# clayne/CPU-Raytracer

Measured on AMD Instinct MI355X. Metric: Mrays/s (primary+shadow+reflection+refraction), higher is better.
Workload: dtype f32

## Files before the change

cpu-raytracer_amd/csrc/rtx_api.hip:

```cpp
#include <hip/hip_runtime.h>
#include <stdio.h>
#include <stdlib.h>
#include <string.h>
#include <math.h>
#include <string>
#include <vector>
#include <algorithm>
#include <type_traits>

#include "../../include/rtx.h"
#include "rtx_device.h"
#include "rtx_math.h"
#include "rtx_libm.h"
#include "rtx_texture.h"
#include "rtx_trace.h"
#include "rtx_shade.h"
#include "rtx_packet.h"
#include "rtx_present.h"
#include "rtx_update.h"
#include "rtx_refit.h"
#include "rtx_build.h"
#include "rtx_normals.h"
#include "rtx_query.h"
#include "rtx_nearest.h"
// ... 31 lines not shown
    hipStream_t stream = nullptr;
    hipStream_t own_stream = nullptr;
    hipStream_t any_stream = nullptr;
    hipEvent_t ev_shade0 = nullptr, ev_shade_last = nullptr, ev_any_done = nullptr;
    void * ext_rgb = nullptr, * ext_packed = nullptr;
    std::string err;
    int n_cu = 0;

    struct BlasRefit { std::vector<int32_t> map4, map4c; bool bound = false; int32_t vertex_count = 0; DevBuf block; DevRefit dev; float * planes[3] = { nullptr, nullptr, nullptr }; void * sort_tmp = nullptr; size_t sort_bytes = 0; };
    struct BlasBuild { bool allocated = false; DevBuf block; DevBuild dev; void * sort_tmp = nullptr; size_t sort_bytes = 0; int levels = 0; };
    struct BlasNormals { bool allocated = false, set = false; DevBuf block; DevNormals dev; void * sort_tmp = nullptr; size_t sort_bytes = 0; unsigned int key_bits = 0; };
    struct BlasSide { bool allocated = false; DevBuf block; DevSide dev; };
    struct BlasHost { std::vector<DevBuf> arrays; int max_local_material = -1, inner_depth = -1; bool packet_ok = true; BlasRefit refit; BlasBuild build; BlasNormals normals; BlasSide side; };
    std::vector<DevBlas> h_blas;
    std::vector<BlasHost> blas;
    DevBuf d_blas, d_materials, d_textures, d_sky, d_ewa;
    std::vector<DevTexture> h_tex;
    std::vector<DevBuf> tex_texels;
    struct TexUpdate { bool allocated = false; rtxt::Plan plan; };
    std::vector<TexUpdate> tex_update;
    DevBuf d_srgb_lut;
    bool sky_uploaded = false;
    int material_count = 0, sky_size = 0;
    std::vector<rtx_material> h_materials; int tlas_inner_depth = -1; std::vector<int> frame_primitive_materials; bool refs_dirty = true; Knobs knobs; int item_blocks = 0, item_cap_alloc = 0; DevBuf d_pk_items, d_pk_item_count;

    DevBuf d_frame;
    StageRing frame_ring;
    DevScene scene;
    bool frame_set = false;
    bool frame_rigid = true;
    LoneFacts frame_lone = { false, false };
    DevBuf d_upd, d_upd_sort; int upd_cap = 0;
    DevBuf d_views, d_vfb_rgb, d_vfb_packed;
    StageRing view_ring;
    int32_t view_count = 0, vfb_cap = 0, ext_vcap = 0;
    void * ext_vrgb = nullptr, * ext_vpacked = nullptr;
    DevBuf d_rays;
    StageRing ray_ring;
    int32_t ray_count = 0, ext_ray_count = 0;
    const void * ext_rays = nullptr;
    uint32_t aov_channels = 0; bool aov_ext = false; int64_t aov_ext_cap = 0; DevAov aov_ext_ptrs = {};
    DevBuf d_aov[8]; int64_t aov_own_cap[8] = {};

    DevQueues q;
    DevBuf qb[20];
    DevBuf d_query[4], d_query_counters, d_query_heads; int32_t query_cap = 0;
    DevBuf d_query_sort; int32_t query_sort_cap = 0; size_t query_sort_tmp = 0;
// ... 119 lines not shown
        if (fc > 0.0) c->pk_blocks_closest = ((int)(c->n_cu * fc) + 1) & ~1;
    }
    {
        const int g = RTX_PK_CLASSES * RTX_WAVE / RTX_PK_BLOCK > 1 ? RTX_PK_CLASSES * RTX_WAVE / RTX_PK_BLOCK : 1;
        c->pk_blocks_any = (c->pk_blocks_any + g - 1) / g * g; c->pk_blocks_closest = (c->pk_blocks_closest + g - 1) / g * g;
        if (c->pk_blocks_any < g) c->pk_blocks_any = g;
        if (c->pk_blocks_closest < g) c->pk_blocks_closest = g;
    }
    long long max_threads = (long long)(c->trace_blocks_closest > c->trace_blocks_any ? c->trace_blocks_closest : c->trace_blocks_any) * RTX_TRACE_BLOCK;
    if ((long long)c->trace_blocks_count * RTX_TRACE_BLOCK > max_threads) max_threads = (long long)c->trace_blocks_count * RTX_TRACE_BLOCK;
    if ((long long)c->pk_blocks_any * RTX_PK_BLOCK > max_threads) max_threads = (long long)c->pk_blocks_any * RTX_PK_BLOCK;
    if ((long long)c->pk_blocks_closest * RTX_PK_BLOCK > max_threads) max_threads = (long long)c->pk_blocks_closest * RTX_PK_BLOCK;
    c->q.pk_defer_t0 = (int)knob_int("RTX_PK_DEFER", 8, 0, 64);
    c->q.pk_defer_leaf = (int)knob_int("RTX_PK_DEFER_LEAF", c->q.pk_defer_t0 / 2, 0, 64);
    c->q.pk_defer_t0_closest = (int)knob_int("RTX_PK_DEFER_CLOSEST", 64, 0, 64);
    c->q.pk_closest_asm = (int)knob_int("RTX_PK_CLOSEST_ASM", 1, 0, 1);
    c->q.pk_defer_t0_primary = (int)knob_int("RTX_PK_DEFER_PRIMARY", c->q.pk_closest_asm ? 4 : 64, 0, 64);
    c->q.pk_order = (int)knob_int("RTX_PK_ORDER", 1, 0, 1);
    c->q.prof_level = (int)knob_int("RTX_LANE_PROF_LEVEL", 2, 0, 100 + RTX_MAX_LEVELS);
    c->q.pk_defer_grow = (int)knob_int("RTX_PK_GROW", 3, 0, 31);
    c->q.spill_threads = (int)max_threads;
    rc = ensure(c, c->d_spill, (size_t)c->q.spill_threads * (RTX_MAX_STACK - RTX_LDS_STACK) * 4 * 3);
    if (!rc) rc = ensure(c, c->d_pk_fifo, (size_t)c->q.spill_threads * RTX_PK_FIFO * 8);
    { int ib = 0; hipOccupancyMaxActiveBlocksPerMultiprocessor(&ib, k_items, RTX_ITEM_BLOCK, 0); c->item_blocks = c->n_cu * (ib > 0 ? ib : 4);
      const double f = knob_real("RTX_ITEM_GRID", 0.0, 0.05, 64.0); if (f > 0.0) c->item_blocks = (int)(c->n_cu * f) > 0 ? (int)(c->n_cu * f) : 1; }
    c->q.pk_items = nullptr; c->q.pk_item_count = nullptr; c->q.pk_item_cap = 0;
    if (rc) { rtx_destroy(c); return rc; }
    bind_tables(c);
    *out_ctx = c;
    return RTX_OK;
}

extern "C" int rtx_destroy(rtx_ctx * c) {
    if (!c) return RTX_ERR_INVALID_ARG;
    hipSetDevice(c->cfg.device);
    if (c->stream) hipStreamSynchronize(c->stream);
    for (hipEvent_t e : c->event_pool) hipEventDestroy(e);
    if (c->graph_exec) { hipGraphExecDestroy(c->graph_exec); c->graph_exec = nullptr; }
    if (c->order_stream) { hipStreamSynchronize(c->order_stream); hipStreamDestroy(c->order_stream); hipEventDestroy(c->ev_cost); hipEventDestroy(c->ev_order); }
    if (c->any_stream) { hipStreamSynchronize(c->any_stream); hipStreamDestroy(c->any_stream); }
    if (c->ev_shade0) hipEventDestroy(c->ev_shade0);
    if (c->ev_shade_last) hipEventDestroy(c->ev_shade_last);
    if (c->ev_any_done) hipEventDestroy(c->ev_any_done);
    if (c->own_stream) hipStreamDestroy(c->own_stream);
    delete c;
    return RTX_OK;
}
// ... 976 lines not shown
        case SHADE_AOV_COUNT: hipLaunchKernelGGL((k_shade<true, false, VW, true, DevAov>),  g, b, 0, c->stream, sc, q, level, aov_t); break;
        case SHADE_AOV_CULL:  hipLaunchKernelGGL((k_shade<false, true, VW, true, DevAov>),  g, b, 0, c->stream, sc, q, level, aov_t); break;
        case SHADE_AOV:       hipLaunchKernelGGL((k_shade<false, false, VW, true, DevAov>), g, b, 0, c->stream, sc, q, level, aov_t); break;
        case SHADE_COUNT:     hipLaunchKernelGGL((k_shade<true, false, VW>),  g, b, 0, c->stream, sc, q, level); break;
        case SHADE_CULL:      hipLaunchKernelGGL((k_shade<false, true, VW>),  g, b, 0, c->stream, sc, q, level); break;
        default:              hipLaunchKernelGGL((k_shade<false, false, VW>), g, b, 0, c->stream, sc, q, level); break;
        }
    }); });
}

static void launch_any(rtx_ctx * c, const AnyLaunch & a, const DevScene & sc, const DevQueues & q) {
    const hipStream_t st = a.stream ? c->any_stream : c->stream;
    const dim3 plain(c->trace_blocks_count), lane(c->trace_blocks_any), tb(RTX_TRACE_BLOCK), pk(c->pk_blocks_any), pb(RTX_PK_BLOCK);
    launch_timed(c, "k_trace_any", st, [&] {
        switch (a.kernel) {
        case ANY_PLAIN_COUNT:   hipLaunchKernelGGL((k_trace<true, true>),   plain, tb, 0, st, sc, q, a.lo); break;
        case ANY_PLAIN:         hipLaunchKernelGGL((k_trace<true, false>),  plain, tb, 0, st, sc, q, a.lo); break;
        case ANY_LANE:          hipLaunchKernelGGL((k_trace_fast<true>),    lane, tb, 0, st, sc, q, a.lo, a.hi); break;
        case ANY_PACKET_STATS:  hipLaunchKernelGGL((k_packet<true, true>),  pk, pb, 0, st, sc, q, a.lo, a.hi); break;
        case ANY_PACKET_SPLIT:  hipLaunchKernelGGL((k_packet<true, false, true>), pk, pb, 0, st, sc, q, a.lo, a.hi); break;
        default:                hipLaunchKernelGGL((k_packet<true, false>), pk, pb, 0, st, sc, q, a.lo, a.hi); break;
        }
    });
    if (a.items) launch_timed(c, "k_trace_items", st, [&] { hipLaunchKernelGGL(k_items, dim3(c->item_blocks), dim3(RTX_ITEM_BLOCK), 0, st, sc, q, c->pk_blocks_any * (RTX_PK_BLOCK / RTX_WAVE), a.lo); });
}

static int run_batch(rtx_ctx * c, const RenderPlan & plan, const DevScene & sc, const DevQueues & q, const DevAov & aov_t, bool first_batch) {
    begin_batch(c, q.counters, q.pk_heads, (uint32_t)q.primary_slots, plan.plain != 0, first_batch);
    if (plan.heatmap) {
        launch_closest(c, plan, sc, q, 0);
        launch_timed(c, "k_heatmap", c->stream, [&] { with_views(plan.views, [&](auto V) { if constexpr (decltype(V)::value != RTX_CAM_RAYS) hipLaunchKernelGGL((k_heatmap<decltype(V)::value>), dim3(plan.stream_blocks), dim3(256), 0, c->stream, sc, q); }); });
        return RTX_OK;
    }
    int next_any = 0;
    for (int level = 0; level < plan.levels; level++) {
        launch_closest(c, plan, sc, q, level);
        if (plan.lpt && level == 0) {
            HIP_OK(c, hipEventRecord(c->ev_cost, c->stream)); HIP_OK(c, hipStreamWaitEvent(c->order_stream, c->ev_cost, 0));
            hipLaunchKernelGGL(k_packet_order, dim3(1), dim3(1024), 0, c->order_stream, (const uint32_t *)c->d_pk_cost.p, (uint32_t *)c->d_pk_order.p, plan.lpt_n);
            HIP_OK(c, hipEventRecord(c->ev_order, c->order_stream));
            c->lpt_valid = true;
        }
        launch_shade(c, plan, sc, q, aov_t, level);
        bool joined = false;
        for (; next_any < plan.n_any && plan.any[next_any].after_level == level; next_any++) {
            if (plan.any[next_any].stream && !joined) {
                const hipEvent_t ev = level == 0 ? c->ev_shade0 : c->ev_shade_last;
// ... 421 lines not shown
    if (rc) return rc;
    hipLaunchKernelGGL(k_debug_texture, dim3((n + 255) / 256), dim3(256), 0, c->stream, sc, texture_id, (const float *)din.p, (float *)dout.p, n);
    HIP_OK(c, hipStreamSynchronize(c->stream));
    HIP_OK(c, hipMemcpy(out3, dout.p, (size_t)n * 12, hipMemcpyDeviceToHost));
    return RTX_OK;
}

__global__ void k_debug_sky(const float * sky, int size, const float * dirs, float * out3, int n) {
    const int i = blockIdx.x * blockDim.x + threadIdx.x;
    if (i >= n) return;
    const v3 r = sky_sample(sky, size, V3(dirs[3 * i], dirs[3 * i + 1], dirs[3 * i + 2]));
    out3[3 * i] = r.x; out3[3 * i + 1] = r.y; out3[3 * i + 2] = r.z;
}

extern "C" int rtx_debug_blas_wide(rtx_ctx * c, int32_t blas_id, int32_t * stack_need) {
    if (!c || !stack_need || blas_id < 0 || (size_t)blas_id >= c->h_blas.size() || !c->h_blas[blas_id].nodes) return RTX_ERR_INVALID_ARG;
    *stack_need = c->h_blas[blas_id].pk4_nodes ? c->h_blas[blas_id].pk4_need : -1;
    return RTX_OK;
}

extern "C" int rtx_debug_blas_wide_closest(rtx_ctx * c, int32_t blas_id, int32_t * stack_need) {
    if (!c || !stack_need || blas_id < 0 || (size_t)blas_id >= c->h_blas.size() || !c->h_blas[blas_id].nodes) return RTX_ERR_INVALID_ARG;
    *stack_need = c->h_blas[blas_id].pk4c_nodes ? c->h_blas[blas_id].pk4c_need : -1;
    return RTX_OK;
}

extern "C" int rtx_debug_grids(rtx_ctx * c, int32_t out[8]) {
    if (!c || !out) return RTX_ERR_INVALID_ARG;
    out[0] = c->n_cu; out[1] = c->trace_blocks_closest; out[2] = c->trace_blocks_any; out[3] = c->trace_blocks_count;
    out[4] = c->pk_blocks_closest; out[5] = c->pk_blocks_any; out[6] = c->item_blocks; out[7] = c->q.spill_threads;
    return RTX_OK;
}

extern "C" int rtx_debug_sky_sample(rtx_ctx * c, const float * dirs3, float * out3, int32_t n) {
    if (!c || !dirs3 || !out3 || n <= 0) return RTX_ERR_INVALID_ARG;
    hipSetDevice(c->cfg.device);
    DevBuf din, dout;
    int rc = upload(c, din, dirs3, (size_t)n * 12);
    if (!rc) rc = ensure(c, dout, (size_t)n * 12);
    if (rc) return rc;
    hipLaunchKernelGGL(k_debug_sky, dim3((n + 255) / 256), dim3(256), 0, c->stream, (const float *)c->d_sky.p, c->sky_size, (const float *)din.p, (float *)dout.p, n);
    HIP_OK(c, hipStreamSynchronize(c->stream));
    HIP_OK(c, hipMemcpy(out3, dout.p, (size_t)n * 12, hipMemcpyDeviceToHost));
    return RTX_OK;
}

// ... 841 lines not shown
```

cpu-raytracer_amd/csrc/rtx_device.h:

```cpp
#pragma once
#include <hip/hip_runtime.h>
#include <stdint.h>
#include "../../include/rtx.h"
#include "rtx_limits.h"

typedef float rtx_f4v __attribute__((ext_vector_type(4)));
typedef const __attribute__((address_space(1))) rtx_f4v * rtx_gptr;
#define RTX_GPTR(p) ((rtx_gptr)(const void *)(p))
static __device__ __forceinline__ float4 gld(rtx_gptr p, int i) { const rtx_f4v v = p[i]; return make_float4(v.x, v.y, v.z, v.w); }
typedef float rtx_f3v __attribute__((ext_vector_type(3)));
static __device__ __forceinline__ float3 gld3(rtx_gptr p, int i) {
    const rtx_f3v v = *(const __attribute__((address_space(1))) rtx_f3v *)(p + i);
    return make_float3(v.x, v.y, v.z);
}

#define RTX_TRI_STRIDE  4
#ifndef RTX_LDS_STACK
#define RTX_LDS_STACK    16
#endif
#define RTX_TRACE_BLOCK  256

#define PRIM_NONE     0
#define PRIM_TRI      (1 << 28)
#define PRIM_SPHERE   (2 << 28)
// ... 103 lines not shown
    int32_t *     pk_fifo;
    int32_t       prof_level;
    int32_t       pk_order;
    int32_t       pk_defer_grow;
    int32_t       pk_closest_asm;
    int32_t       pk_defer_t0_primary;
    int32_t       pk_defer_t0_closest;
    int32_t       pk_defer_t0;
    int32_t       pk_defer_leaf;
    int32_t       pk_item_cap;
    uint4 *       pk_items;
    uint32_t *    pk_item_count;
    DevCounters * counters;
    uint32_t *    stats_partial;
    int32_t       stats_stride;
    int32_t       stats_n[RTX_MAX_LEVELS + 1];
    uint32_t *       pk_cost;
    const uint32_t * pk_lpt_order;
    uint32_t *    pk_heads;
    uint32_t *    tm_packed;
    int32_t       tm_base;
    float *       fb_rgb;
    uint32_t *    fb_packed;
};
```

cpu-raytracer_amd/csrc/rtx_packet.h:

```cpp
#pragma once
#include "rtx_math.h"
#include "rtx_device.h"
#include "rtx_trace.h"
#include "rtx_shade.h"

#define RTX_PK_CLASSES  8
#ifndef RTX_PK_WAVES_ANY
#define RTX_PK_WAVES_ANY 5
#endif
#ifndef RTX_PK_WAVES_SPLIT
#define RTX_PK_WAVES_SPLIT 5
#endif
#ifndef RTX_PK_WAVES_CLOSEST
#define RTX_PK_WAVES_CLOSEST 4
#endif
#ifndef RTX_PK_CHUNK
#define RTX_PK_CHUNK 64u
#endif
#ifndef RTX_PK_WAVES_FUSED
#define RTX_PK_WAVES_FUSED 3
#endif

typedef const __attribute__((address_space(4))) rtx_f4v * rtx_cptr;
typedef float rtx_f2v __attribute__((ext_vector_type(2)));
// ... 1752 lines not shown
    if (lane == 0) for (int i = 0; i < 10; i++) { if (i == 4 || i == 5 || i == 7 || i == 8 || i == 9) atomicMax(&ctr->work[(ANY ? 0 : 10) + i], W.prof[i]); else atomicAdd(&ctr->work[(ANY ? 0 : 10) + i], W.prof[i]); }
#endif
#ifdef RTX_LANE_PROF
    if (!ANY && level == q.prof_level % 100 && lane == 0 && (W.lp[12] > 0u || (q.prof_level >= 100 && lp_had_packet))) {
        for (int i = 0; i < 10; i++) atomicAdd(&ctr->work[i], (unsigned long long)W.lp[i]);
        atomicMax(&ctr->work[10], (unsigned long long)W.lp[10]); atomicMax(&ctr->work[11], (unsigned long long)W.lp[11]); atomicAdd(&ctr->work[12], (unsigned long long)W.lp[12]);
        atomicMax(&ctr->work[13], __builtin_amdgcn_s_memtime() - lp_k0);
        atomicAdd(&ctr->work[14], __builtin_amdgcn_s_memtime() - lp_k0);
        atomicAdd(&ctr->work[15], 1ull);
        atomicAdd(&ctr->work[16], __builtin_amdgcn_s_memrealtime() - lp_r0);
        atomicAdd(&ctr->work[17], (unsigned long long)W.lp[13]); atomicAdd(&ctr->work[18], (unsigned long long)W.lp[14]);
        atomicAdd(&ctr->work[19], (unsigned long long)W.lp[15]);
    }
#endif
    if (ANY && SPLIT && q.pk_items && lane == 0) { q.pk_item_count[gwave] = (uint32_t)W.item_n; if ((uint32_t)W.item_n > __hip_atomic_load(&ctr->item_max[level], __ATOMIC_RELAXED, __HIP_MEMORY_SCOPE_AGENT)) atomicMax(&ctr->item_max[level], (uint32_t)W.item_n); }
    if (W.err) { if (lane == 0) atomicOr(&ctr->error_flags, ERR_STACK_OVERFLOW); }
    if (PSTAT && lane == 0) {
        atomicAdd(&ctr->work[15 + PKS_PACKETS], st_packets); atomicAdd(&ctr->work[15 + PKS_PAIR_STEPS], W.st_pairs);
        atomicAdd(&ctr->work[15 + PKS_TRI_STEPS], W.st_tris); atomicAdd(&ctr->work[15 + PKS_PAIR_LANES], W.st_pair_lanes);
        atomicAdd(&ctr->work[15 + PKS_TRI_LANES], W.st_tri_lanes);
    }
}

#define RTX_ITEM_LDS 8
#ifndef RTX_ITEM_BLOCK
#define RTX_ITEM_BLOCK 64
#endif
#define RTX_ITEM_MESHES 32
#ifndef RTX_ITEM_WAVES
#define RTX_ITEM_WAVES 6
#endif
__global__ __launch_bounds__(RTX_ITEM_BLOCK, RTX_ITEM_WAVES)
void k_items(const DevScene sc, const DevQueues q, const int n_chunks, const int level) {
    __shared__ int s_stk[RTX_ITEM_LDS][RTX_ITEM_BLOCK];
    __shared__ unsigned long long s_mesh[RTX_ITEM_MESHES][2];
    for (int b = threadIdx.x; b < RTX_ITEM_MESHES && b < sc.blas_count; b += blockDim.x) { s_mesh[b][0] = (unsigned long long)sc.blas[b].pk4_nodes; s_mesh[b][1] = (unsigned long long)sc.blas[b].tri_hot; }
    __syncthreads();
    const uint32_t gwave = (uint32_t)rfl((int)(blockIdx.x * (RTX_ITEM_BLOCK / RTX_WAVE) + (threadIdx.x >> 6)));
    const uint32_t n_batches = ((uint32_t)rfl((int)q.counters->item_max[level]) + 63u) >> 6;
    const uint32_t nwaves = gridDim.x * (RTX_ITEM_BLOCK / RTX_WAVE), units = (uint32_t)n_chunks * n_batches;
    int ovf[RTX_PK4_MAX_NEED + 4];
#ifdef RTX_ITEM_STATS
    unsigned long long st_iters = 0, st_busy = 0, st_batches = 0, st_items = 0;
#endif
    uint32_t u = gwave, pos = 0, lim = 0; const uint4 * items = q.pk_items;
    auto next_unit = [&]() {
        for (; u < units; u += nwaves) {
            const uint32_t chunk = u % (uint32_t)n_chunks, first = (u / (uint32_t)n_chunks) * 64u;
            const uint32_t n = (uint32_t)rfl((int)q.pk_item_count[chunk]);
            if (first < n) { pos = first; lim = first + 64u < n ? first + 64u : n; items = q.pk_items + 3 * (size_t)chunk * (size_t)q.pk_item_cap; u += nwaves; return true; }
        }
        return false;
    };
    bool have_unit = next_unit();
    bool busy = false, have_cur = false; uint32_t slot = 0; int psp = 0, cur_first = 0, cur_cnt = 0;
    v3 co = V3(0.0f, 0.0f, 0.0f), cd = V3(1.0f, 1.0f, 1.0f);
    PkRay ray; pk_set_ray(ray, co, cd, cd); ray.tcur = 0.0f;
    rtx_gptr nodes4 = nullptr, tris = nullptr;
    auto push = [&](int e) { if (psp < RTX_ITEM_LDS) s_stk[psp][threadIdx.x] = e; else if (psp < RTX_ITEM_LDS + RTX_PK4_MAX_NEED + 4) ovf[psp - RTX_ITEM_LDS] = e; psp++; };
    for (;;) {
        const unsigned long long idle = __ballot(!busy);
        if (idle != 0ull && have_unit) {
            const uint32_t rank = (uint32_t)__builtin_amdgcn_mbcnt_hi((uint32_t)(idle >> 32), __builtin_amdgcn_mbcnt_lo((uint32_t)idle, 0u));
            const uint32_t take = (uint32_t)__popcll(idle), avail = lim - pos;
            if (!busy && rank < avail) {
                const uint4 * const it = items + 3 * (size_t)(pos + rank);
                const uint4 q0 = it[0], q1 = it[1]; const uint2 q2 = *(const uint2 *)(it + 2);
                slot = q1.w;
                if (q2.y < RTX_ITEM_MESHES) { nodes4 = (rtx_gptr)s_mesh[q2.y][0]; tris = (rtx_gptr)s_mesh[q2.y][1]; }
                else { const DevBlas & B = sc.blas[q2.y]; nodes4 = RTX_GPTR(B.pk4_nodes); tris = RTX_GPTR(B.tri_hot); }
                co = V3(as_f((int)q0.x), as_f((int)q0.y), as_f((int)q0.z)); cd = V3(as_f((int)q1.x), as_f((int)q1.y), as_f((int)q1.z));
                pk_set_ray(ray, co, cd, vrcp(cd)); ray.tcur = as_f((int)q0.w);
                cur_first = rtxl::wide_first((int)q2.x); cur_cnt = rtxl::wide_count((int)q2.x); have_cur = true; psp = 0;
                busy = q.socc[slot] == 0u;
#ifdef RTX_ITEM_STATS
                st_items++;
#endif
            }
            pos += take < avail ? take : avail;
            if (pos >= lim) have_unit = next_unit();
        }
        if (__ballot(busy) == 0ull) { if (!have_unit) break; else continue; }
#ifdef RTX_ITEM_STATS
        st_iters++; st_busy += (unsigned long long)__popcll(__ballot(busy));
#endif
        if (busy && have_cur && cur_cnt == 0) {
            const Pk4Step s = pk4_step(nodes4, cur_first, ray);
            if (s.q3) push(s.e3);
            if (s.q2) push(s.e2);
            if (s.q1) push(s.e1);
            have_cur = s.have_cur; cur_first = s.cur_first; cur_cnt = s.cur_cnt;
        }
        if (busy && have_cur && cur_cnt > 0) {
            have_cur = false;
            for (int t = cur_first; t < cur_first + cur_cnt; t++) {
                const float4 p0 = gld(tris, RTX_TRI_STRIDE * t), e1 = gld(tris, RTX_TRI_STRIDE * t + 1), e2 = gld(tris, RTX_TRI_STRIDE * t + 2);
                float tt, uu, vv;
                if (tri_test(v3q(p0), v3q(e1), v3q(e2), co, cd, ray.tcur, tt, uu, vv)) { q.socc[slot] = 1u; busy = false; break; }
            }
        }
        if (busy && !have_cur) {
            if (psp == 0) busy = false;
            else {
                psp--;
                const int e = psp < RTX_ITEM_LDS ? s_stk[psp][threadIdx.x] : ovf[psp - RTX_ITEM_LDS];
                cur_first = rtxl::wide_first(e); cur_cnt = rtxl::wide_count(e); have_cur = true;
            }
        }
    }
#ifdef RTX_ITEM_STATS
    if ((threadIdx.x & 63) == 0) { atomicAdd(&q.counters->work[16], st_iters); atomicAdd(&q.counters->work[17], st_busy); atomicMax(&q.counters->work[19], st_iters); }
    atomicAdd(&q.counters->work[15], st_items);
#endif
}
```

cpu-raytracer_amd/csrc/rtx_plan.h:

```cpp
#pragma once
#include <stdint.h>
#include <string.h>
#include "../../include/rtx.h"
#include "rtx_limits.h"

struct Knobs {
    long long slot_budget;
    long long item_bytes_max;
    int shade_grid;
    int lane_from_level;
    int lane_from_level_any;
    int split_items;
    int resolve_block;
    int pk4_order;
    bool merge_any, no_wide, no_wide_closest, fail_item_alloc, graph; int lpt;
    bool fuse_shade;
    int update_small_max;
    int tex_pass_levels;
    bool lone_entry;
};

struct LoneFacts { bool lone, copy_class; };
static inline LoneFacts plan_lone_facts(int instance_count, const rtx_bvh_node * tlas_nodes, int tlas_node_count, const int32_t * tlas_indices, int tlas_index_count,
                                        const rtx_instance * instances) {
    LoneFacts f = { false, false };
    if (instance_count != 1 || tlas_node_count < 1 || tlas_index_count < 1 || !tlas_nodes || !tlas_indices || !instances) return f;
    if (tlas_nodes[0].count != 1 || tlas_nodes[0].left_or_first != 0 || tlas_indices[0] != 0) return f;
    f.lone = true;
    uint32_t bits[12]; memcpy(bits, instances[0].world_inv, sizeof(bits));
    f.copy_class = true;
    for (int k = 0; k < 12; k++) {
        const bool diagonal = k == 0 || k == 5 || k == 10;
        if (diagonal ? bits[k] != 0x3f800000u : (bits[k] & 0x7fffffffu) != 0u) f.copy_class = false;
    }
    return f;
}

struct StackFigures { bool unfit_mesh; int dt, blas_any, blas_shared; };

static inline bool plan_can_spawn(const rtx_material * materials, size_t count) {
    for (size_t i = 0; i < count; i++)
        for (int a = 0; a < 3; a++) if (materials[i].reflection[a] != 0.0f || materials[i].transmittance[a] != 0.0f) return true;
// ... 143 lines not shown
```

cpu-raytracer_amd/pyrtx/api.py:

```python
from __future__ import annotations

import ctypes as C
import os
from typing import Dict, List, Optional

import numpy as np

from . import scene_io as sio
from .ctypes_structs import RtxConfig, RtxFrame, RtxStats, RtxWork, RtxTextureDesc, RtxAovBuffers, RtxRay, RtxQueryFilter, AOV_CHANNELS, RTX_AOV_ALL, fill_frame

_HERE = os.path.dirname(os.path.abspath(__file__))
LIB_PATH = os.path.join(_HERE, "..", "csrc", "librtx_hip.so")

EXPORTS = ["rtx_abi_version", "rtx_create", "rtx_destroy", "rtx_last_error", "rtx_upload_blas", "rtx_upload_materials",
           "rtx_upload_texture", "rtx_upload_sky", "rtx_set_frame", "rtx_render_tiles", "rtx_synchronize", "rtx_get_stats",
           "rtx_read_framebuffer", "rtx_framebuffer_device_ptrs", "rtx_last_kernel_times", "rtx_enable_kernel_timing",
           "rtx_bind_framebuffer", "rtx_set_stream", "rtx_present", "rtx_debug_libm", "rtx_debug_texture_sample", "rtx_debug_sky_sample", "rtx_debug_blas_wide", "rtx_debug_blas_wide_closest",
           "rtx_group_unique_id", "rtx_group_create", "rtx_group_render", "rtx_group_destroy", "rtx_group_attach", "rtx_group_create_local", "rtx_group_render_local",
           "rtx_group_layout", "rtx_group_slot_pixels", "rtx_debug_group_loopback", "rtx_debug_trace_rays", "rtx_debug_occluded", "rtx_debug_light_plot",
           "rtx_set_views", "rtx_render_views", "rtx_read_views", "rtx_bind_view_framebuffer", "rtx_bind_aovs", "rtx_read_aovs",
           "rtx_set_rays", "rtx_bind_rays", "rtx_render_rays", "rtx_update_instances", "rtx_read_frame_state",
           "rtx_bind_blas_vertices", "rtx_refit_blas", "rtx_read_blas", "rtx_alloc_blas", "rtx_build_blas",
           "rtx_query_closest", "rtx_query_occluded", "rtx_debug_query_order", "rtx_debug_read_layouts",
           "rtx_alloc_texture", "rtx_update_texture", "rtx_read_texture", "rtx_update_sky",
           "rtx_alloc_blas_topology", "rtx_set_blas_topology", "rtx_blas_vertex_normals", "rtx_query_nearest", "rtx_query_hits", "rtx_query_sweep",
           "rtx_debug_grids", "rtx_set_object_masks", "rtx_update_object_masks", "rtx_read_object_masks",
           "rtx_query_nearest_filtered", "rtx_query_hits_filtered", "rtx_query_sweep_filtered",
           "rtx_blas_pseudonormals", "rtx_read_blas_pseudonormals", "rtx_query_signed_distance",
           "rtx_query_overlap", "rtx_query_overlap_filtered", "rtx_query_sweep_box", "rtx_query_sweep_box_filtered",
           "rtx_query_overlap_capsule", "rtx_query_overlap_capsule_filtered"]
VIEW_EXPORTS = ("rtx_set_views", "rtx_render_views", "rtx_read_views", "rtx_bind_view_framebuffer")
AOV_EXPORTS = ("rtx_bind_aovs", "rtx_read_aovs")
RAY_EXPORTS = ("rtx_set_rays", "rtx_bind_rays", "rtx_render_rays")
UPDATE_EXPORTS = ("rtx_update_instances", "rtx_read_frame_state")
REFIT_EXPORTS = ("rtx_bind_blas_vertices", "rtx_refit_blas", "rtx_read_blas")
BUILD_EXPORTS = ("rtx_alloc_blas", "rtx_build_blas")
QUERY_EXPORTS = ("rtx_query_closest", "rtx_query_occluded")
QUERY_SORT_EXPORTS = ("rtx_debug_query_order",)
LAYOUT_EXPORTS = ("rtx_debug_read_layouts",)
TEXTURE_EXPORTS = ("rtx_alloc_texture", "rtx_update_texture", "rtx_read_texture", "rtx_update_sky")
NORMALS_EXPORTS = ("rtx_alloc_blas_topology", "rtx_set_blas_topology", "rtx_blas_vertex_normals")
NEAREST_EXPORTS = ("rtx_query_nearest",)
SIGNED_EXPORTS = ("rtx_blas_pseudonormals", "rtx_read_blas_pseudonormals", "rtx_query_signed_distance")
HITS_EXPORTS = ("rtx_query_hits",)
SWEEP_EXPORTS = ("rtx_query_sweep",)
GRID_EXPORTS = ("rtx_debug_grids",)
MASK_EXPORTS = ("rtx_set_object_masks", "rtx_update_object_masks", "rtx_read_object_masks",
                "rtx_query_nearest_filtered", "rtx_query_hits_filtered", "rtx_query_sweep_filtered")
OVERLAP_EXPORTS = ("rtx_query_overlap", "rtx_query_overlap_filtered")
SWEEP_BOX_EXPORTS = ("rtx_query_sweep_box", "rtx_query_sweep_box_filtered")
OVERLAP_CAPSULE_EXPORTS = ("rtx_query_overlap_capsule", "rtx_query_overlap_capsule_filtered")
OPTIONAL_EXPORTS = (OVERLAP_CAPSULE_EXPORTS + SWEEP_BOX_EXPORTS + OVERLAP_EXPORTS + VIEW_EXPORTS + AOV_EXPORTS + RAY_EXPORTS + UPDATE_EXPORTS + REFIT_EXPORTS + QUERY_EXPORTS + QUERY_SORT_EXPORTS + LAYOUT_EXPORTS
                    + TEXTURE_EXPORTS + NORMALS_EXPORTS + NEAREST_EXPORTS + HITS_EXPORTS + SWEEP_EXPORTS + GRID_EXPORTS + MASK_EXPORTS + SIGNED_EXPORTS)
RTX_QUERY_MAX_HITS = 8
RTX_TEXELS_RGB_F32 = 0
RTX_TEXELS_RGBA8_SRGB = 1
RTX_UPDATE_MAX_INSTANCES = 65536
RTX_ERR_STATE = 5

RTX_RENDER_COUNT_WORK = 1
RTX_RENDER_SIMPLE_TRACE = 2
RTX_RENDER_CULL_DEAD_SHADOW_RAYS = 4
RTX_RENDER_SERIAL = 8
RTX_RENDER_LANE_TRACE = 16
RTX_RENDER_PACKET_STATS = 32
RTX_RENDER_PACKET_CLOSEST = 64
RTX_RENDER_AOV = 128
RTX_MAX_VIEWS = 4096
RTX_QUERY_DISTANCE = 1
RTX_QUERY_POSITION = 2
RTX_QUERY_NORMAL = 4
RTX_QUERY_UV = 16
RTX_QUERY_MATERIAL_ID = 32
RTX_QUERY_OBJECT_ID = 64
RTX_QUERY_TRIANGLE_ID = 128
# ... 93 lines not shown
        lib.rtx_build_blas.argtypes = [vp, i32, vp, vp, vp, vp, vp]
    if hasattr(lib, "rtx_query_closest"):
        lib.rtx_query_closest.argtypes = [vp, vp, C.c_int64, u32, C.POINTER(RtxQueryBuffers), u32]
        lib.rtx_query_occluded.argtypes = [vp, vp, C.c_int64, vp, u32]
    if hasattr(lib, "rtx_query_nearest"):
        lib.rtx_query_nearest.argtypes = [vp, vp, C.c_int64, u32, C.POINTER(RtxQueryBuffers), u32]
    if hasattr(lib, "rtx_query_sweep"):
        lib.rtx_query_sweep.argtypes = [vp, vp, C.c_int64, u32, C.POINTER(RtxQueryBuffers), u32]
    if hasattr(lib, "rtx_query_hits"):
        lib.rtx_query_hits.argtypes = [vp, vp, C.c_int64, i32, u32, C.POINTER(RtxQueryBuffers), vp, u32]
    if hasattr(lib, "rtx_set_object_masks"):
        lib.rtx_set_object_masks.argtypes = [vp, vp, i32]
        lib.rtx_update_object_masks.argtypes = [vp, vp, i32]
        lib.rtx_read_object_masks.argtypes = [vp, vp, i32, C.POINTER(i32)]
        lib.rtx_query_nearest_filtered.argtypes = [vp, vp, C.c_int64, u32, C.POINTER(RtxQueryBuffers), u32, C.POINTER(RtxQueryFilter)]
        lib.rtx_query_sweep_filtered.argtypes = [vp, vp, C.c_int64, u32, C.POINTER(RtxQueryBuffers), u32, C.POINTER(RtxQueryFilter)]
        lib.rtx_query_hits_filtered.argtypes = [vp, vp, C.c_int64, i32, u32, C.POINTER(RtxQueryBuffers), vp, u32, C.POINTER(RtxQueryFilter)]
    if hasattr(lib, "rtx_debug_query_order"):
        lib.rtx_debug_query_order.argtypes = [vp, vp, i32, C.c_int64, vp]
    if hasattr(lib, "rtx_debug_read_layouts"):
        lib.rtx_debug_read_layouts.argtypes = [vp, i32, vp, vp, vp, vp, vp, vp, vp]
    if hasattr(lib, "rtx_debug_grids"):
        lib.rtx_debug_grids.argtypes = [vp, vp]
    if hasattr(lib, "rtx_update_texture"):
        lib.rtx_alloc_texture.argtypes = [vp, i32, i32, i32, i32]
        lib.rtx_update_texture.argtypes = [vp, i32, vp, i32]
        lib.rtx_read_texture.argtypes = [vp, i32, C.POINTER(RtxTextureDesc), vp, C.c_int64]
        lib.rtx_update_sky.argtypes = [vp, vp, i32]
    if hasattr(lib, "rtx_blas_vertex_normals"):
        lib.rtx_alloc_blas_topology.argtypes = [vp, i32, i32, i32]
        lib.rtx_set_blas_topology.argtypes = [vp, i32, vp]
        lib.rtx_blas_vertex_normals.argtypes = [vp, i32, vp, vp]
    if hasattr(lib, "rtx_query_signed_distance"):
        lib.rtx_blas_pseudonormals.argtypes = [vp, i32, vp]
        lib.rtx_read_blas_pseudonormals.argtypes = [vp, i32, vp, vp]
        lib.rtx_query_signed_distance.argtypes = [vp, vp, C.c_int64, u32, C.POINTER(RtxQueryBuffers), vp, vp, u32, C.POINTER(RtxQueryFilter)]
    if hasattr(lib, "rtx_query_overlap"):
        lib.rtx_query_overlap.argtypes = [vp, vp, C.c_int64, i32, vp, vp, vp, u32]
        lib.rtx_query_overlap_filtered.argtypes = [vp, vp, C.c_int64, i32, vp, vp, vp, u32, C.POINTER(RtxQueryFilter)]
    if hasattr(lib, "rtx_query_overlap_capsule"):
        lib.rtx_query_overlap_capsule.argtypes = [vp, vp, C.c_int64, i32, vp, vp, vp, u32]
        lib.rtx_query_overlap_capsule_filtered.argtypes = [vp, vp, C.c_int64, i32, vp, vp, vp, u32, C.POINTER(RtxQueryFilter)]
    if hasattr(lib, "rtx_query_sweep_box"):
        lib.rtx_query_sweep_box.argtypes = [vp, vp, C.c_int64, vp, vp, vp, vp, vp, u32]
        lib.rtx_query_sweep_box_filtered.argtypes = [vp, vp, C.c_int64, vp, vp, vp, vp, vp, u32, C.POINTER(RtxQueryFilter)]
    for name in EXPORTS:
# ... 761 lines not shown
    def debug_read_layouts(self, blas_id: int = -1) -> Dict:
        info = np.zeros(8, np.int32)
        self._chk(self.lib.rtx_debug_read_layouts(self.ctx, int(blas_id), info.ctypes.data, None, None, None, None, None, None), "rtx_debug_read_layouts")
        n = int(info[0])
        pk = np.zeros((n, 8), np.uint32)
        if blas_id < 0:
            self._chk(self.lib.rtx_debug_read_layouts(self.ctx, int(blas_id), None, pk.ctypes.data, None, None, None, None, None), "rtx_debug_read_layouts")
            return {"pk": pk}
        pk4 = np.zeros((2 * n + 4, 8), np.uint32) if info[1] else None
        pk4c = np.zeros((2 * n + 4, 8), np.uint32) if info[2] else None
        planes = [np.zeros(int(info[3 + a]), np.uint32) for a in range(3)]
        self._chk(self.lib.rtx_debug_read_layouts(self.ctx, int(blas_id), None, pk.ctypes.data, None if pk4 is None else pk4.ctypes.data,
                                                  None if pk4c is None else pk4c.ctypes.data, *(p.ctypes.data if p.size else None for p in planes)),
                  "rtx_debug_read_layouts")
        return {"pk": pk, "pk4": pk4, "pk4c": pk4c, "planes": planes}

    GRID_NAMES = ("cus", "trace_blocks_closest", "trace_blocks_any", "trace_blocks_count", "pk_blocks_closest", "pk_blocks_any", "item_blocks",
                  "spill_threads")

    def debug_grids(self) -> np.ndarray:
        out = np.zeros(8, np.int32)
        self._chk(self.lib.rtx_debug_grids(self.ctx, out.ctypes.data), "rtx_debug_grids")
        return out

    def _query_rows(self, name: str, rows, width: int, n: Optional[int]):
        if isinstance(rows, (int, np.integer)) and not isinstance(rows, bool):
            if n is None:
                raise ValueError(f"n is needed when {name} is a raw device pointer")
            if int(n) < 1 or not rows:
                raise ValueError(f"{name}: a non-null device pointer and n >= 1 are needed, not {rows} and {n}")
            return int(rows), int(n), None
        import torch
        if not isinstance(rows, torch.Tensor):
            raise TypeError(f"{name} must be a torch.Tensor (or a raw device pointer with n), not {type(rows).__name__}")
        if rows.dtype != torch.float32:
            raise TypeError(f"{name} must be torch.float32, not {rows.dtype}")
        if rows.dim() != 2 or rows.shape[1] != width:
            raise ValueError(f"{name} must have shape (n, {width}), not {tuple(rows.shape)}")
        if not rows.is_contiguous():
            raise ValueError(f"{name} must be contiguous")
        if n is None:
            n = int(rows.shape[0])
        if not 1 <= int(n) <= rows.shape[0]:
            raise ValueError(f"n must be in [1, {rows.shape[0]}] for {name} of shape {tuple(rows.shape)}, not {n}")
        return rows.data_ptr(), int(n), rows

# ... 500 lines not shown
```

include/rtx.h:

```cpp
#ifndef RTX_H
#define RTX_H

#include <stdint.h>

#ifdef __cplusplus
extern "C" {
#endif

#define RTX_ABI_VERSION 1

enum {
    RTX_OK               = 0,
    RTX_ERR_INVALID_ARG  = 1,
    RTX_ERR_NO_DEVICE    = 2,
    RTX_ERR_HIP          = 3,
    RTX_ERR_LIMIT        = 4,
    RTX_ERR_STATE        = 5,
    RTX_ERR_OOM          = 6
};

enum { RTX_TRAVERSE_NAIVE = 0, RTX_TRAVERSE_ORDERED = 1 };
enum { RTX_TEXTURE_NEAREST = 0, RTX_TEXTURE_BILINEAR = 1, RTX_TEXTURE_MIPMAP = 2 };
enum { RTX_MIP_TRILINEAR = 0, RTX_MIP_ANISOTROPIC = 1, RTX_MIP_EWA = 2 };

// ... 335 lines not shown
int rtx_group_unique_id(void * id128);
int rtx_group_create(rtx_ctx * ctx, int32_t rank, int32_t world, const void * id128, rtx_group ** out_group);
int rtx_group_render(rtx_group * group, uint32_t flags);
int rtx_group_destroy(rtx_group * group);
int rtx_group_attach(rtx_ctx * ctx, rtx_group * base, rtx_group ** out_group);
int rtx_group_create_local(rtx_ctx ** contexts, int32_t n, rtx_group ** out_groups);
int rtx_group_render_local(rtx_group ** groups, int32_t n, uint32_t flags);
int rtx_group_layout(int32_t width, int32_t height, int32_t world, int32_t rank, int32_t * tiles_total, int32_t * tiles_per_rank, int32_t * own_tiles);
int rtx_group_slot_pixels(int32_t width, int32_t height, int32_t world, int32_t rank, int64_t * pixel_index, int64_t capacity);


int rtx_debug_libm(rtx_ctx * ctx, int32_t fn, const float * a, const float * b, float * out, int32_t n);
int rtx_debug_texture_sample(rtx_ctx * ctx, int32_t texture_id, const float * in6, float * out_rgb, int32_t n);
int rtx_debug_trace_rays(rtx_ctx * ctx, const float * rays18, int32_t n, float * hits27, uint32_t flags);
int rtx_debug_occluded(rtx_ctx * ctx, const float * origin_direction_maxdist7, int32_t n, uint32_t * occluded, uint32_t flags);
int rtx_debug_light_plot(rtx_ctx * ctx, const rtx_point_light * pl, const rtx_spot_light * sl, const rtx_directional_light * dl,
                         const float * in10, float * out9, int32_t n_light, const float * rgb, uint32_t * packed, int32_t n_plot);
int rtx_debug_group_loopback(rtx_ctx * ctx, int32_t world, uint32_t flags);
int rtx_debug_blas_wide(rtx_ctx * ctx, int32_t blas_id, int32_t * stack_need);
int rtx_debug_blas_wide_closest(rtx_ctx * ctx, int32_t blas_id, int32_t * stack_need);
int rtx_debug_read_layouts(rtx_ctx * ctx, int32_t blas_id, int32_t * info8, float * pk_nodes, float * pk4_nodes, float * pk4c_nodes,
                           float * planes_x, float * planes_y, float * planes_z);
int rtx_debug_grids(rtx_ctx * ctx, int32_t out[8]);
int rtx_debug_sky_sample(rtx_ctx * ctx, const float * directions_xyz, float * out_rgb, int32_t n);

#ifdef __cplusplus
}
#endif
#endif
```

Baseline: 9981.

## Add intra-wave work stealing and multi-round refill to item traversal kernel

Templates the k_items any-hit kernel on a STEAL flag, enabled by default. Idle lanes now redraw items over several ballot rounds when a drawn item is already occluded. Once the global item queue is drained, busy lanes donate a traversal stack entry plus their ray state to idle lanes via ds_bpermute. The aim is to cut lane idleness and tail divergence in the any-hit wave loop, at the cost of extra ballots, shared-memory exchange, register pressure and an optional debug counter.

Result: no change. 9949 (-0.3%).

```diff
diff --git a/cpu-raytracer_amd/csrc/rtx_api.hip b/cpu-raytracer_amd/csrc/rtx_api.hip
--- a/cpu-raytracer_amd/csrc/rtx_api.hip
+++ b/cpu-raytracer_amd/csrc/rtx_api.hip
@@ -77,7 +77,7 @@
     DevBuf d_srgb_lut;
     bool sky_uploaded = false;
     int material_count = 0, sky_size = 0;
-    std::vector<rtx_material> h_materials; int tlas_inner_depth = -1; std::vector<int> frame_primitive_materials; bool refs_dirty = true; Knobs knobs; int item_blocks = 0, item_cap_alloc = 0; DevBuf d_pk_items, d_pk_item_count;
+    std::vector<rtx_material> h_materials; int tlas_inner_depth = -1; std::vector<int> frame_primitive_materials; bool refs_dirty = true; Knobs knobs; int item_blocks = 0, item_cap_alloc = 0; DevBuf d_pk_items, d_pk_item_count, d_item_dbg;
 
     DevBuf d_frame;
     StageRing frame_ring;
@@ -243,7 +243,10 @@
     c->q.spill_threads = (int)max_threads;
     rc = ensure(c, c->d_spill, (size_t)c->q.spill_threads * (RTX_MAX_STACK - RTX_LDS_STACK) * 4 * 3);
     if (!rc) rc = ensure(c, c->d_pk_fifo, (size_t)c->q.spill_threads * RTX_PK_FIFO * 8);
-    { int ib = 0; hipOccupancyMaxActiveBlocksPerMultiprocessor(&ib, k_items, RTX_ITEM_BLOCK, 0); c->item_blocks = c->n_cu * (ib > 0 ? ib : 4);
+    K.item_steal = knob_int("RTX_ITEM_STEAL", 1, 0, 1) != 0;
+    if (!rc) rc = ensure(c, c->d_item_dbg, sizeof(unsigned long long));
+    if (!rc) { hipMemset(c->d_item_dbg.p, 0, sizeof(unsigned long long)); c->q.item_dbg = knob_int("RTX_ITEM_STEAL_DEBUG", 0, 0, 1) != 0 ? (unsigned long long *)c->d_item_dbg.p : nullptr; }
+    { int ib = 0; if (K.item_steal) hipOccupancyMaxActiveBlocksPerMultiprocessor(&ib, k_items<true>, RTX_ITEM_BLOCK, 0); else hipOccupancyMaxActiveBlocksPerMultiprocessor(&ib, k_items<false>, RTX_ITEM_BLOCK, 0); c->item_blocks = c->n_cu * (ib > 0 ? ib : 4);
       const double f = knob_real("RTX_ITEM_GRID", 0.0, 0.05, 64.0); if (f > 0.0) c->item_blocks = (int)(c->n_cu * f) > 0 ? (int)(c->n_cu * f) : 1; }
     c->q.pk_items = nullptr; c->q.pk_item_count = nullptr; c->q.pk_item_cap = 0;
     if (rc) { rtx_destroy(c); return rc; }
@@ -1266,7 +1269,7 @@
         default:                hipLaunchKernelGGL((k_packet<true, false>), pk, pb, 0, st, sc, q, a.lo, a.hi); break;
         }
     });
-    if (a.items) launch_timed(c, "k_trace_items", st, [&] { hipLaunchKernelGGL(k_items, dim3(c->item_blocks), dim3(RTX_ITEM_BLOCK), 0, st, sc, q, c->pk_blocks_any * (RTX_PK_BLOCK / RTX_WAVE), a.lo); });
+    if (a.items) launch_timed(c, "k_trace_items", st, [&] { hipLaunchKernelGGL(HIP_KERNEL_NAME(c->knobs.item_steal ? k_items<true> : k_items<false>), dim3(c->item_blocks), dim3(RTX_ITEM_BLOCK), 0, st, sc, q, c->pk_blocks_any * (RTX_PK_BLOCK / RTX_WAVE), a.lo); });
 }
 
 static int run_batch(rtx_ctx * c, const RenderPlan & plan, const DevScene & sc, const DevQueues & q, const DevAov & aov_t, bool first_batch) {
@@ -1734,6 +1737,16 @@
 extern "C" int rtx_debug_blas_wide_closest(rtx_ctx * c, int32_t blas_id, int32_t * stack_need) {
     if (!c || !stack_need || blas_id < 0 || (size_t)blas_id >= c->h_blas.size() || !c->h_blas[blas_id].nodes) return RTX_ERR_INVALID_ARG;
     *stack_need = c->h_blas[blas_id].pk4c_nodes ? c->h_blas[blas_id].pk4c_need : -1;
+    return RTX_OK;
+}
+
+extern "C" int rtx_debug_item_steals(rtx_ctx * c, uint64_t out[2]) {
+    if (!c || !out) return RTX_ERR_INVALID_ARG;
+    hipSetDevice(c->cfg.device);
+    unsigned long long w = 0;
+    HIP_OK(c, hipMemcpyAsync(&w, c->d_item_dbg.p, sizeof(w), hipMemcpyDeviceToHost, c->stream));
+    HIP_OK(c, hipStreamSynchronize(c->stream));
+    out[0] = w >> 32; out[1] = w & 0xffffffffull;
     return RTX_OK;
 }
 
diff --git a/cpu-raytracer_amd/csrc/rtx_device.h b/cpu-raytracer_amd/csrc/rtx_device.h
--- a/cpu-raytracer_amd/csrc/rtx_device.h
+++ b/cpu-raytracer_amd/csrc/rtx_device.h
@@ -149,4 +149,5 @@
     int32_t       tm_base;
     float *       fb_rgb;
     uint32_t *    fb_packed;
+    unsigned long long * item_dbg;
 };
diff --git a/cpu-raytracer_amd/csrc/rtx_packet.h b/cpu-raytracer_amd/csrc/rtx_packet.h
--- a/cpu-raytracer_amd/csrc/rtx_packet.h
+++ b/cpu-raytracer_amd/csrc/rtx_packet.h
@@ -1798,6 +1798,12 @@
     }
 }
 
+#ifndef RTX_ITEM_ROUNDS
+#define RTX_ITEM_ROUNDS 2
+#endif
+#ifndef RTX_ITEM_STEAL_IDLE
+#define RTX_ITEM_STEAL_IDLE 16
+#endif
 #define RTX_ITEM_LDS 8
 #ifndef RTX_ITEM_BLOCK
 #define RTX_ITEM_BLOCK 64
@@ -1806,9 +1812,11 @@
 #ifndef RTX_ITEM_WAVES
 #define RTX_ITEM_WAVES 6
 #endif
+template <bool STEAL>
 __global__ __launch_bounds__(RTX_ITEM_BLOCK, RTX_ITEM_WAVES)
 void k_items(const DevScene sc, const DevQueues q, const int n_chunks, const int level) {
     __shared__ int s_stk[RTX_ITEM_LDS][RTX_ITEM_BLOCK];
+    __shared__ int s_xch[RTX_ITEM_BLOCK];
     __shared__ unsigned long long s_mesh[RTX_ITEM_MESHES][2];
     for (int b = threadIdx.x; b < RTX_ITEM_MESHES && b < sc.blas_count; b += blockDim.x) { s_mesh[b][0] = (unsigned long long)sc.blas[b].pk4_nodes; s_mesh[b][1] = (unsigned long long)sc.blas[b].tri_hot; }
     __syncthreads();
@@ -1834,10 +1842,70 @@
     PkRay ray; pk_set_ray(ray, co, cd, cd); ray.tcur = 0.0f;
     rtx_gptr nodes4 = nullptr, tris = nullptr;
     auto push = [&](int e) { if (psp < RTX_ITEM_LDS) s_stk[psp][threadIdx.x] = e; else if (psp < RTX_ITEM_LDS + RTX_PK4_MAX_NEED + 4) ovf[psp - RTX_ITEM_LDS] = e; psp++; };
+    uint32_t n_steal = 0, n_redraw = 0;
+    const int lane = (int)(threadIdx.x & 63u), xbase = (int)(threadIdx.x & ~63u);
+    auto lane_rank = [&](unsigned long long m) { return (uint32_t)__builtin_amdgcn_mbcnt_hi((uint32_t)(m >> 32), __builtin_amdgcn_mbcnt_lo((uint32_t)m, 0u)); };
     for (;;) {
         const unsigned long long idle = __ballot(!busy);
-        if (idle != 0ull && have_unit) {
-            const uint32_t rank = (uint32_t)__builtin_amdgcn_mbcnt_hi((uint32_t)(idle >> 32), __builtin_amdgcn_mbcnt_lo((uint32_t)idle, 0u));
+        if (STEAL && idle != 0ull && have_unit) {
+            bool want = !busy, fresh = false; uint32_t mesh = 0;
+            for (int round = 0; round < RTX_ITEM_ROUNDS; round++) {
+                const unsigned long long wm = __ballot(want);
+                if (wm == 0ull || !have_unit) break;
+                const uint32_t rank = lane_rank(wm), take = (uint32_t)__popcll(wm), avail = lim - pos;
+                if (want && rank < avail) {
+                    const uint4 * const it = items + 3 * (size_t)(pos + rank);
+                    const uint4 q0 = it[0], q1 = it[1]; const uint2 q2 = *(const uint2 *)(it + 2);
+                    slot = q1.w; mesh = q2.y;
+                    co = V3(as_f((int)q0.x), as_f((int)q0.y), as_f((int)q0.z)); cd = V3(as_f((int)q1.x), as_f((int)q1.y), as_f((int)q1.z));
+                    ray.tcur = as_f((int)q0.w);
+                    cur_first = rtxl::wide_first((int)q2.x); cur_cnt = rtxl::wide_count((int)q2.x);
+                    if (q.socc[slot] == 0u) { want = false; fresh = true; }
+#ifdef RTX_ITEM_STATS
+                    st_items++;
+#endif
+                }
+                const uint32_t drew = take < avail ? take : avail;
+                if (round > 0) n_redraw += drew;
+                pos += drew;
+                if (pos >= lim) have_unit = next_unit();
+            }
+            if (fresh) {
+                if (mesh < RTX_ITEM_MESHES) { nodes4 = (rtx_gptr)s_mesh[mesh][0]; tris = (rtx_gptr)s_mesh[mesh][1]; }
+                else { const DevBlas & B = sc.blas[mesh]; nodes4 = RTX_GPTR(B.pk4_nodes); tris = RTX_GPTR(B.tri_hot); }
+                pk_set_ray(ray, co, cd, vrcp(cd));
+                have_cur = true; psp = 0; busy = true;
+            }
+        }
+        if (STEAL && !have_unit) {
+            const unsigned long long tm = __ballot(!busy);
+            const bool donor = busy && psp >= 1 && psp <= RTX_ITEM_LDS;
+            const unsigned long long dm = __popcll(tm) >= RTX_ITEM_STEAL_IDLE ? __ballot(donor) : 0ull;
+            if (dm != 0ull) {
+                const uint32_t nd = (uint32_t)__popcll(dm), nt = (uint32_t)__popcll(tm), n = nd < nt ? nd : nt;
+                const bool give = donor && lane_rank(dm) < n, takes = !busy && lane_rank(tm) < n;
+                int e = 0;
+                if (give) { psp--; e = s_stk[psp][threadIdx.x]; s_xch[xbase + (int)lane_rank(dm)] = lane; }
+                __builtin_amdgcn_fence(__ATOMIC_RELEASE, "wavefront"); __builtin_amdgcn_wave_barrier(); __builtin_amdgcn_fence(__ATOMIC_ACQUIRE, "wavefront");
+                const int src = (takes ? s_xch[xbase + (int)lane_rank(tm)] : lane) << 2;
+                auto xf = [&](float v) { return as_f(__builtin_amdgcn_ds_bpermute(src, as_i(v))); };
+                auto xi = [&](int v) { return __builtin_amdgcn_ds_bpermute(src, v); };
+                const int te = xi(e), tslot = xi((int)slot);
+                const v3 to = V3(xf(co.x), xf(co.y), xf(co.z)), td = V3(xf(cd.x), xf(cd.y), xf(cd.z));
+                const v3 ti = V3(xf(ray.i_xy.x), xf(ray.i_xy.y), xf(ray.i_zz.x)); const float tt = xf(ray.tcur);
+                const unsigned long long an = (unsigned long long)nodes4, at = (unsigned long long)tris;
+                const uint32_t n_lo = (uint32_t)xi((int)(uint32_t)an), n_hi = (uint32_t)xi((int)(uint32_t)(an >> 32)), t_lo = (uint32_t)xi((int)(uint32_t)at), t_hi = (uint32_t)xi((int)(uint32_t)(at >> 32));
+                if (takes) {
+                    slot = (uint32_t)tslot; co = to; cd = td; pk_set_ray(ray, to, td, ti); ray.tcur = tt;
+                    nodes4 = (rtx_gptr)(((unsigned long long)n_hi << 32) | n_lo); tris = (rtx_gptr)(((unsigned long long)t_hi << 32) | t_lo);
+                    cur_first = rtxl::wide_first(te); cur_cnt = rtxl::wide_count(te); have_cur = true; psp = 0;
+                    busy = q.socc[slot] == 0u;
+                }
+                n_steal += n;
+            }
+        }
+        if (!STEAL && idle != 0ull && have_unit) {
+            const uint32_t rank = lane_rank(idle);
             const uint32_t take = (uint32_t)__popcll(idle), avail = lim - pos;
             if (!busy && rank < avail) {
                 const uint4 * const it = items + 3 * (size_t)(pos + rank);
@@ -1884,8 +1952,10 @@
             }
         }
     }
+    if (STEAL && q.item_dbg && lane == 0 && (n_steal | n_redraw) != 0u) atomicAdd(q.item_dbg, ((unsigned long long)n_steal << 32) | (unsigned long long)n_redraw);
 #ifdef RTX_ITEM_STATS
-    if ((threadIdx.x & 63) == 0) { atomicAdd(&q.counters->work[16], st_iters); atomicAdd(&q.counters->work[17], st_busy); atomicMax(&q.counters->work[19], st_iters); }
+    if ((threadIdx.x & 63) == 0) { atomicAdd(&q.counters->work[16], st_iters); atomicAdd(&q.counters->work[17], st_busy); atomicMax(&q.counters->work[19], st_iters);
+                                   atomicAdd(&q.counters->work[18], ((unsigned long long)n_steal << 32) | (unsigned long long)n_redraw); }
     atomicAdd(&q.counters->work[15], st_items);
 #endif
 }
diff --git a/cpu-raytracer_amd/csrc/rtx_plan.h b/cpu-raytracer_amd/csrc/rtx_plan.h
--- a/cpu-raytracer_amd/csrc/rtx_plan.h
+++ b/cpu-raytracer_amd/csrc/rtx_plan.h
@@ -18,6 +18,7 @@
     int update_small_max;
     int tex_pass_levels;
     bool lone_entry;
+    bool item_steal;
 };
 
 struct LoneFacts { bool lone, copy_class; };
diff --git a/cpu-raytracer_amd/pyrtx/api.py b/cpu-raytracer_amd/pyrtx/api.py
--- a/cpu-raytracer_amd/pyrtx/api.py
+++ b/cpu-raytracer_amd/pyrtx/api.py
@@ -28,7 +28,7 @@
            "rtx_query_nearest_filtered", "rtx_query_hits_filtered", "rtx_query_sweep_filtered",
            "rtx_blas_pseudonormals", "rtx_read_blas_pseudonormals", "rtx_query_signed_distance",
            "rtx_query_overlap", "rtx_query_overlap_filtered", "rtx_query_sweep_box", "rtx_query_sweep_box_filtered",
-           "rtx_query_overlap_capsule", "rtx_query_overlap_capsule_filtered"]
+           "rtx_query_overlap_capsule", "rtx_query_overlap_capsule_filtered", "rtx_debug_item_steals"]
 VIEW_EXPORTS = ("rtx_set_views", "rtx_render_views", "rtx_read_views", "rtx_bind_view_framebuffer")
 AOV_EXPORTS = ("rtx_bind_aovs", "rtx_read_aovs")
 RAY_EXPORTS = ("rtx_set_rays", "rtx_bind_rays", "rtx_render_rays")
@@ -45,12 +45,13 @@
 HITS_EXPORTS = ("rtx_query_hits",)
 SWEEP_EXPORTS = ("rtx_query_sweep",)
 GRID_EXPORTS = ("rtx_debug_grids",)
+ITEM_EXPORTS = ("rtx_debug_item_steals",)
 MASK_EXPORTS = ("rtx_set_object_masks", "rtx_update_object_masks", "rtx_read_object_masks",
                 "rtx_query_nearest_filtered", "rtx_query_hits_filtered", "rtx_query_sweep_filtered")
 OVERLAP_EXPORTS = ("rtx_query_overlap", "rtx_query_overlap_filtered")
 SWEEP_BOX_EXPORTS = ("rtx_query_sweep_box", "rtx_query_sweep_box_filtered")
 OVERLAP_CAPSULE_EXPORTS = ("rtx_query_overlap_capsule", "rtx_query_overlap_capsule_filtered")
-OPTIONAL_EXPORTS = (OVERLAP_CAPSULE_EXPORTS + SWEEP_BOX_EXPORTS + OVERLAP_EXPORTS + VIEW_EXPORTS + AOV_EXPORTS + RAY_EXPORTS + UPDATE_EXPORTS + REFIT_EXPORTS + QUERY_EXPORTS + QUERY_SORT_EXPORTS + LAYOUT_EXPORTS
+OPTIONAL_EXPORTS = (ITEM_EXPORTS + OVERLAP_CAPSULE_EXPORTS + SWEEP_BOX_EXPORTS + OVERLAP_EXPORTS + VIEW_EXPORTS + AOV_EXPORTS + RAY_EXPORTS + UPDATE_EXPORTS + REFIT_EXPORTS + QUERY_EXPORTS + QUERY_SORT_EXPORTS + LAYOUT_EXPORTS
                     + TEXTURE_EXPORTS + NORMALS_EXPORTS + NEAREST_EXPORTS + HITS_EXPORTS + SWEEP_EXPORTS + GRID_EXPORTS + MASK_EXPORTS + SIGNED_EXPORTS)
 RTX_QUERY_MAX_HITS = 8
 RTX_TEXELS_RGB_F32 = 0
@@ -190,6 +191,8 @@
         lib.rtx_debug_read_layouts.argtypes = [vp, i32, vp, vp, vp, vp, vp, vp, vp]
     if hasattr(lib, "rtx_debug_grids"):
         lib.rtx_debug_grids.argtypes = [vp, vp]
+    if hasattr(lib, "rtx_debug_item_steals"):
+        lib.rtx_debug_item_steals.argtypes = [vp, vp]
     if hasattr(lib, "rtx_update_texture"):
         lib.rtx_alloc_texture.argtypes = [vp, i32, i32, i32, i32]
         lib.rtx_update_texture.argtypes = [vp, i32, vp, i32]
@@ -997,6 +1000,11 @@
         out = np.zeros(8, np.int32)
         self._chk(self.lib.rtx_debug_grids(self.ctx, out.ctypes.data), "rtx_debug_grids")
         return out
+
+    def debug_item_steals(self) -> tuple:
+        out = np.zeros(2, np.uint64)
+        self._chk(self.lib.rtx_debug_item_steals(self.ctx, out.ctypes.data), "rtx_debug_item_steals")
+        return int(out[0]), int(out[1])
 
     def _query_rows(self, name: str, rows, width: int, n: Optional[int]):
         if isinstance(rows, (int, np.integer)) and not isinstance(rows, bool):
diff --git a/include/rtx.h b/include/rtx.h
--- a/include/rtx.h
+++ b/include/rtx.h
@@ -381,6 +381,7 @@
 int rtx_debug_read_layouts(rtx_ctx * ctx, int32_t blas_id, int32_t * info8, float * pk_nodes, float * pk4_nodes, float * pk4c_nodes,
                            float * planes_x, float * planes_y, float * planes_z);
 int rtx_debug_grids(rtx_ctx * ctx, int32_t out[8]);
+int rtx_debug_item_steals(rtx_ctx * ctx, uint64_t out[2]);
 int rtx_debug_sky_sample(rtx_ctx * ctx, const float * directions_xyz, float * out_rgb, int32_t n);
 
 #ifdef __cplusplus
```
